# dalcinl/PetIGA

Hardware: NVIDIA B200
Metric: assembled_Mnnz_per_s (higher is better)
Workload: dtype f64

## Files before the change

### petiga_b200/csrc/pc_api.cu

```cuda
#include <dlfcn.h>

#include <sched.h>

#include <algorithm>
#include <cctype>
#include <cstdio>
#include <cstdio>
#include <cstring>
#include <string>
#include <vector>

#include "pc_plan.h"

namespace pc {

namespace {
typedef int (*nvtx_push_t)(const char*);
typedef int (*nvtx_pop_t)(void);
nvtx_push_t g_nvtx_push = nullptr;
nvtx_pop_t g_nvtx_pop = nullptr;
int g_nvtx_state = 0;
const char* const kSlotNames[PETIGA_NSLOTS] = {"IGAComputeVector", "IGAComputeMatrix", "IGAComputeSystem", "IGAComputeFunction", "IGAComputeJacobian",
                                               "IGAComputeIFunction", "IGAComputeIJacobian", "IGAComputeIEFunction", "IGAComputeIEJacobian",
                                               "IGAComputeRHSFunction", "IGAComputeRHSJacobian", "IGAComputeI2Function", "IGAComputeI2Jacobian"};
// ... 169 lines not shown
    part[2 * blockIdx.x] = x; part[2 * blockIdx.x + 1] = y;
  }
}

__global__ void __launch_bounds__(256) dfma_peak_kernel(double* out, int iters, double a, double b) {
  double x0 = threadIdx.x, x1 = x0 + 1, x2 = x0 + 2, x3 = x0 + 3, x4 = x0 + 4, x5 = x0 + 5, x6 = x0 + 6, x7 = x0 + 7;
  for (int i = 0; i < iters; i++) {
#pragma unroll
    for (int k = 0; k < 8; k++) {
      x0 = fma(x0, a, b); x1 = fma(x1, a, b); x2 = fma(x2, a, b); x3 = fma(x3, a, b);
      x4 = fma(x4, a, b); x5 = fma(x5, a, b); x6 = fma(x6, a, b); x7 = fma(x7, a, b);
    }
  }
  const double s = ((x0 + x1) + (x2 + x3)) + ((x4 + x5) + (x6 + x7));
  if (s == 12345.678) out[0] = s;
}

}

using namespace pc;

extern "C" {

int petiga_cuda_version(void) { return PETIGA_CUDA_VERSION; }

const char* petiga_cuda_strerror(int code) {
  switch (code) {
    case PETIGA_CUDA_OK: return "success";
    case PETIGA_CUDA_ERR_ARG: return "invalid argument";
    case PETIGA_CUDA_ERR_ORDER: return "operation called out of order";
    case PETIGA_CUDA_ERR_SUP: return "configuration not supported by the device path";
    case PETIGA_CUDA_ERR_MEM: return "out of memory";
    case PETIGA_CUDA_ERR_CUDA: return "CUDA runtime error";
    case PETIGA_CUDA_ERR_NODEVICE: return "no CUDA device (libpetiga_cuda has no CPU fallback)";
    case PETIGA_CUDA_ERR_NCCL: return "NCCL error";
  }
  return "unknown error";
}

const char* petiga_cuda_last_error(void) { return g_last_error.c_str(); }

int petiga_cuda_device_count(int* count) {
  int n = 0;
  cudaError_t e = cudaGetDeviceCount(&n);
  if (count) *count = (e == cudaSuccess) ? n : 0;
  if (e != cudaSuccess) return cuda_fail(e, "cudaGetDeviceCount");
  return n > 0 ? 0 : PETIGA_CUDA_ERR_NODEVICE;
}

int petiga_cuda_plan_create(petiga_cuda_plan** plan, const petiga_cuda_space* sp, int rank, int nranks, void* nccl_comm,
                            void* stream, int device) {
  if (!plan || !sp) return PETIGA_CUDA_ERR_ARG;
  *plan = nullptr;
  int ndev = 0;
  int rc = petiga_cuda_device_count(&ndev);
  if (rc) { if (g_last_error.empty()) set_error("no CUDA device; libpetiga_cuda has no CPU fallback"); return rc; }
  if (device < 0 || device >= ndev) { set_error("bad device ordinal"); return PETIGA_CUDA_ERR_ARG; }
  petiga_cuda_plan* P = new (std::nothrow) petiga_cuda_plan();
  if (!P) return PETIGA_CUDA_ERR_MEM;
  memset(&P->bc, 0, sizeof(P->bc));
  rc = build_layout(*sp, rank, nranks, P->L);
  if (rc) { set_error(P->L.error); delete P; return rc; }
  if (sp->order < 1 || sp->order > 4) { set_error("order must be in [1,4]"); delete P; return PETIGA_CUDA_ERR_ARG; }
  P->order = sp->order;
  P->device = device;
  P->nccl = nccl_comm;
  auto bail = [&](int code) { petiga_cuda_plan_destroy(P); return code; };
  if (cudaSetDevice(device) != cudaSuccess) return bail(cuda_fail(cudaGetLastError(), "cudaSetDevice"));
  if (stream) P->stream = (cudaStream_t)stream;
  else {
    cudaError_t e = cudaStreamCreateWithFlags(&P->stream, cudaStreamNonBlocking);
    if (e != cudaSuccess) return bail(cuda_fail(e, "cudaStreamCreate"));
    P->own_stream = true;
  }
  cudaDeviceGetAttribute(&P->num_sms, cudaDevAttrMultiProcessorCount, device);
  cudaEventCreate(&P->ev0);
  cudaEventCreate(&P->ev1);
  const Layout& L = P->L;
  for (int d = 0; d < 3; d++) {
    const AxisLayout& a = L.ax[d];
    DevAxis& da = P->dax[d];
    const size_t nq = (size_t)a.nel * a.nqp;
    if (!sp->value[d] || !sp->weight[d] || !sp->point[d] || !sp->detJac[d]) { set_error("missing basis tables"); return bail(PETIGA_CUDA_ERR_ARG); }
    double *v, *w, *pt, *dj; int *off, *W, *lo, *simp; uint32_t* seg;
    if ((rc = upload(P, sp->value[d], nq * (a.p + 1) * 5, &v))) return bail(rc);
    if ((rc = upload(P, sp->weight[d], nq, &w))) return bail(rc);
    if ((rc = upload(P, sp->point[d], nq, &pt))) return bail(rc);
    if ((rc = upload(P, sp->detJac[d], (size_t)a.nel, &dj))) return bail(rc);
    if ((rc = upload(P, sp->offset[d], (size_t)a.nel, &off))) return bail(rc);
    if ((rc = upload(P, a.W.data(), a.W.size(), &W))) return bail(rc);
    if ((rc = upload(P, a.lo.data(), a.lo.size(), &lo))) return bail(rc);
    if ((rc = upload(P, a.seg.data(), a.seg.size(), &seg))) return bail(rc);
    if ((rc = upload(P, a.simple.data(), a.simple.size(), &simp))) return bail(rc);
    da.value = v; da.weight = w; da.point = pt; da.detJac = dj; da.offset = off; da.W = W; da.lo = lo; da.seg = seg; da.simple = simp;
    da.nel = a.nel; da.nqp = a.nqp; da.nen = a.p + 1; da.p = a.p; da.gs = a.gs; da.gw = a.gw; da.es = a.es; da.ew = a.ew;
    da.periodic = a.periodic; da.nnp = a.nnp;
    P->detJac_h[d].assign(sp->detJac[d], sp->detJac[d] + a.nel);
    if ((rc = upload(P, L.rowG[d].data(), L.rowG[d].size(), &P->d_rowG[d]))) return bail(rc);
    if ((rc = upload(P, a.first.data(), a.first.size(), &P->d_first[d]))) return bail(rc);
    if ((rc = upload(P, a.own.data(), a.own.size(), &P->d_own[d]))) return bail(rc);
    if ((rc = upload(P, a.box_ls.data(), a.box_ls.size(), &P->d_box_ls[d]))) return bail(rc);
    if ((rc = upload(P, a.box_lw.data(), a.box_lw.size(), &P->d_box_lw[d]))) return bail(rc);
  }
  if ((rc = upload(P, L.localrow.data(), L.localrow.size(), &P->d_localrow))) return bail(rc);
  if ((rc = upload(P, L.rowbase.data(), L.rowbase.size(), &P->d_rowbase))) return bail(rc);
  if ((rc = upload(P, L.rank_start.data(), L.rank_start.size(), &P->d_rank_start))) return bail(rc);
  if (L.nranks > 1) {
    const size_t nl = (size_t)L.nloc * L.dof;
    if ((rc = upload<double>(P, nullptr, nl, &P->d_rhs_loc))) return bail(rc);
    if ((rc = upload<double>(P, nullptr, nl, &P->d_U_loc))) return bail(rc);
    if ((rc = upload<double>(P, nullptr, nl, &P->d_V_loc))) return bail(rc);
    if ((rc = upload<double>(P, nullptr, nl, &P->d_W_loc))) return bail(rc);
    std::vector<int> rows;
    std::vector<int64_t> offs;
    P->recv_row_off.clear();
    for (auto& r : L.recv) {
      P->recv_row_off.push_back(rows.size());
      rows.insert(rows.end(), r.rows.begin(), r.rows.end());
      int64_t o = 0;
      for (int row : r.rows) { offs.push_back(o); o += L.rowbase[row + 1] - L.rowbase[row]; }
    }
    P->recv_row_off.push_back(rows.size());
    if ((rc = upload(P, rows.data(), rows.size(), &P->d_recv_rows))) return bail(rc);
    if ((rc = upload(P, offs.data(), offs.size(), &P->d_recv_off))) return bail(rc);
  }
  cudaError_t e = cudaStreamSynchronize(P->stream);
  if (e != cudaSuccess) return bail(cuda_fail(e, "plan upload"));
  *plan = P;
  return 0;
}

int petiga_cuda_plan_destroy(petiga_cuda_plan* P) {
  if (!P) return 0;
  cudaSetDevice(P->device);
  if (P->stream) cudaStreamSynchronize(P->stream);
  for (void* d : P->allocs) cudaFree(d);
  for (int b = 0; b < 2; b++) { cudaFree(P->d_rowptr[b]); cudaFree(P->d_colidx[b]); }
  cudaFree(P->d_X); cudaFree(P->d_W); cudaFree(P->d_fixtable); cudaFree(P->d_ghost_values); cudaFree(P->d_recv);
  cudaFree(P->d_scalar); cudaFree(P->d_sf3_dprime); cudaFree(P->d_solve_work); cudaFree(P->d_solve_xfull); cudaFree(P->d_values_own); cudaFree(P->d_rhs_own); cudaFree(P->d_U_own); cudaFree(P->d_V_own);
  if (P->h_pinned) cudaFreeHost(P->h_pinned);
  if (P->ev0) cudaEventDestroy(P->ev0);
  if (P->ev1) cudaEventDestroy(P->ev1);
  if (P->own_stream && P->stream) cudaStreamDestroy(P->stream);
  delete P;
  return 0;
}

int petiga_cuda_set_option(petiga_cuda_plan* P, const char* name, double value) {
  if (!P || !name) return PETIGA_CUDA_ERR_ARG;
  if (!strcmp(name, "path")) { int v = (int)value; if (v < 0 || v > 2) return PETIGA_CUDA_ERR_ARG; P->path = v; return 0; }
  if (!strcmp(name, "scatter")) { P->scatter = (int)value; return 0; }
  if (!strcmp(name, "quad_impl")) { int v = (int)value; if (v < -1 || v > 3) return PETIGA_CUDA_ERR_ARG; P->quad_impl = v; return 0; }
  if (!strcmp(name, "kron_minb_rows")) { P->kron_minb_rows = (int)value; P->config_version++; return 0; }
  if (!strcmp(name, "kron_bulk")) { P->kron_bulk = value != 0; P->config_version++; return 0; }
  if (!strcmp(name, "sf3_static")) { P->sf3_static = value != 0; return 0; }
  if (!strcmp(name, "sf3_variant")) { int v = (int)value; if (v < 0 || v > 1) return PETIGA_CUDA_ERR_ARG; P->sf3_variant = v; return 0; }
  set_error(std::string("unknown option ") + name);
  return PETIGA_CUDA_ERR_ARG;
}

int petiga_cuda_get_stat(petiga_cuda_plan* P, const char* name, double* value) {
  if (!P || !name || !value) return PETIGA_CUDA_ERR_ARG;
  if (!strcmp(name, "launches")) { *value = (double)P->launches; return 0; }
  if (!strcmp(name, "last_path")) { *value = (double)P->last_path; return 0; }
  if (!strcmp(name, "last_impl")) { *value = (double)P->last_impl; return 0; }
  if (!strcmp(name, "last_sf3_static")) { *value = (double)P->last_sf3_static; return 0; }
  if (!strcmp(name, "last_sf3_variant")) { *value = (double)P->last_sf3_variant; return 0; }
  if (!strcmp(name, "last_kernel_ms")) { *value = P->last_kernel_ms; return 0; }
  if (!strcmp(name, "last_flops")) { *value = P->last_flops; return 0; }
  if (!strcmp(name, "num_sms")) { *value = P->num_sms; return 0; }
  if (!strcmp(name, "nghostrows")) { *value = P->L.nghostrows; return 0; }
  if (!strcmp(name, "nnz_loc")) { *value = (double)P->L.nnz_loc; return 0; }
  return PETIGA_CUDA_ERR_ARG;
}

int petiga_cuda_set_geometry(petiga_cuda_plan* P, int nsd, const double* X, const double* W) {
  if (!P) return PETIGA_CUDA_ERR_ARG;
  PC_CUDA(cudaSetDevice(P->device));
  PC_CUDA(cudaStreamSynchronize(P->stream));
  cudaFree(P->d_X); cudaFree(P->d_W);
  P->d_X = P->d_W = nullptr;
  P->config_version++;
  if (!X) return 0;
  if (nsd != P->L.dim) { set_error("geometry: nsd must equal dim on the device path (manifolds unsupported)"); return PETIGA_CUDA_ERR_SUP; }
  const size_t ng = P->L.localrow.size();
  PC_CUDA(cudaMalloc(&P->d_X, ng * nsd * sizeof(double)));
  PC_CUDA(cudaMemcpy(P->d_X, X, ng * nsd * sizeof(double), cudaMemcpyHostToDevice));
  if (W) {
    PC_CUDA(cudaMalloc(&P->d_W, ng * sizeof(double)));
    PC_CUDA(cudaMemcpy(P->d_W, W, ng * sizeof(double), cudaMemcpyHostToDevice));
  }
  return 0;
}

int petiga_cuda_set_bc(petiga_cuda_plan* P, const petiga_cuda_bc* bc) {
  if (!P) return PETIGA_CUDA_ERR_ARG;
  PC_CUDA(cudaSetDevice(P->device));
  PC_CUDA(cudaStreamSynchronize(P->stream));
  cudaFree(P->d_fixtable);
  P->d_fixtable = nullptr;
  P->has_bc = false;
  P->config_version++;
  memset(&P->bc, 0, sizeof(P->bc));
  if (!bc) return 0;
  for (int d = 0; d < 3; d++)
    for (int s = 0; s < 2; s++) {
      if (bc->vcount[d][s] < 0 || bc->vcount[d][s] > 64 || bc->lcount[d][s] < 0 || bc->lcount[d][s] > 64) return PETIGA_CUDA_ERR_ARG;
      if (d < P->L.dim && (bc->vcount[d][s] || bc->lcount[d][s])) P->has_bc = true;
    }
  for (int d = 0; d < 3; d++)
    for (int s = 0; s < 2; s++) {
      for (int k = 0; k < bc->vcount[d][s]; k++) {
        const int f = bc->vfield[d][s][k];
        if (f < 0) { memset(&P->bc, 0, sizeof(P->bc)); P->has_bc = false; set_error("set_bc: negative field index"); return PETIGA_CUDA_ERR_ARG; }
        int pos = -1;
        for (int j = 0; j < P->bc.vcount[d][s]; j++) if (P->bc.vfield[d][s][j] == f) pos = j;
        if (pos < 0) pos = P->bc.vcount[d][s]++;
        P->bc.vfield[d][s][pos] = f; P->bc.vvalue[d][s][pos] = bc->vvalue[d][s][k];
      }
      for (int k = 0; k < bc->lcount[d][s]; k++) {
        const int f = bc->lfield[d][s][k];
        if (f < 0) { memset(&P->bc, 0, sizeof(P->bc)); P->has_bc = false; set_error("set_bc: negative field index"); return PETIGA_CUDA_ERR_ARG; }
        int pos = -1;
        for (int j = 0; j < P->bc.lcount[d][s]; j++) if (P->bc.lfield[d][s][j] == f) pos = j;
        if (pos < 0) pos = P->bc.lcount[d][s]++;
        P->bc.lfield[d][s][pos] = f; P->bc.lvalue[d][s][pos] = bc->lvalue[d][s][k];
      }
    }
  P->bc.fixtableU = nullptr;
  if (bc->fixtableU) {
    const size_t n = P->L.localrow.size() * P->L.dof;
    PC_CUDA(cudaMalloc(&P->d_fixtable, n * sizeof(double)));
    PC_CUDA(cudaMemcpy(P->d_fixtable, bc->fixtableU, n * sizeof(double), cudaMemcpyHostToDevice));
  }
  return 0;
}

int petiga_cuda_set_fixtable_device(petiga_cuda_plan* P, const double* table_own) {
  if (!P) return PETIGA_CUDA_ERR_ARG;
  PC_CUDA(cudaSetDevice(P->device));
  PC_CUDA(cudaStreamSynchronize(P->stream));
  cudaFree(P->d_fixtable);
  P->d_fixtable = nullptr;
  P->config_version++;
  if (!table_own) return 0;
  const Layout& L = P->L;
  const size_t ng = L.localrow.size();
  PC_CUDA(cudaMalloc(&P->d_fixtable, ng * L.dof * sizeof(double)));
  const double* loc = table_own;
  double* tmp = nullptr;
  if (L.nranks > 1) {
    PC_CUDA(cudaMalloc(&tmp, (size_t)L.nloc * L.dof * sizeof(double)));
    int rc = halo_state(P, table_own, tmp);
    if (rc) { cudaFree(tmp); return rc; }
    loc = tmp;
  }
  const int blocks = (int)std::min<size_t>((ng * L.dof + 255) / 256, (size_t)P->num_sms * 8);
  fixtable_scatter_kernel<<<std::max(blocks, 1), 256, 0, P->stream>>>(P->d_localrow, loc, P->d_fixtable, ng, L.dof);
  PC_CUDA(cudaGetLastError());
  P->launches++;
  PC_CUDA(cudaStreamSynchronize(P->stream));
  cudaFree(tmp);
  return 0;
}

int petiga_cuda_form_select(petiga_cuda_plan* P, int slot, int form_id, const double* params, int nparams) {
  if (P && slot >= 0 && slot < PETIGA_NSLOTS && form_id == -1) {
    P->slots[slot].form = -1;
    P->config_version++;
    return 0;
  }
  if (!P || slot < 0 || slot >= PETIGA_NSLOTS || form_id < 0 || form_id >= PETIGA_NFORMS || nparams < 0 || nparams > kMaxPrm) {
    set_error("form_select: bad slot / form / nparams");
    return PETIGA_CUDA_ERR_ARG;
  }
  FormInfo fi = form_info(form_id, slot, P->L.dim, P->L.dof);
  if (!fi.valid) { set_error("form_select: this built-in form does not provide that slot for this dim/dof (PETSC_ERR_SUP)"); return PETIGA_CUDA_ERR_SUP; }
  P->slots[slot].form = form_id;
  P->config_version++;
  memset(P->slots[slot].prm, 0, sizeof(P->slots[slot].prm));
  for (int k = 0; k < nparams; k++) P->slots[slot].prm[k] = params[k];
  return 0;
}

int petiga_cuda_plan_sizes(petiga_cuda_plan* P, int* nown, int* nghost, int64_t* nnzb) {
  if (!P) return PETIGA_CUDA_ERR_ARG;
  if (nown) *nown = P->L.nown;
  if (nghost) *nghost = (int)P->L.localrow.size();
  if (nnzb) *nnzb = P->L.nnz_own;
  return 0;
}

int petiga_cuda_plan_lgmap_host(petiga_cuda_plan* P, int* lgmap) {
  if (!P || !lgmap) return PETIGA_CUDA_ERR_ARG;
  memcpy(lgmap, P->L.lgmap.data(), P->L.lgmap.size() * sizeof(int));
  return 0;
}

int petiga_cuda_plan_pattern(petiga_cuda_plan* P, int block, int* nrows, int64_t* nnz, const int** d_rowptr, const int** d_colidx) {
  if (!P || (block != 0 && block != 1)) return PETIGA_CUDA_ERR_ARG;
  const Layout& L = P->L;
  const int bs = block ? 1 : L.dof;
  const int64_t n = L.nnz_own * bs * bs;
  if (n > INT32_MAX) { set_error("pattern: more than 2^31-1 nonzeros on one rank; use the block (BAIJ) layout or more ranks"); return PETIGA_CUDA_ERR_SUP; }
  PC_CUDA(cudaSetDevice(P->device));
  if (!P->d_rowptr[block]) {
    std::vector<int> rp((size_t)L.nown * bs + 1);
// ... 378 lines not shown
```

### petiga_b200/csrc/pc_kron.cu

```cuda
#include <algorithm>
#include <cstdlib>
#include <cstring>

#include "pc_plan.h"

namespace pc {

namespace {

constexpr int kMaxTerms = 40;
constexpr int kKronP = 4;
constexpr int kMaxWW = (2 * kKronP + 1) * (2 * kKronP + 1);
constexpr int kStageCap = 32 * 16 + 192;

struct KronTerm { unsigned char ij, rs0, rs1, rs2; double c; };
struct KronVTerm { unsigned char i, r0, r1, r2; double c; };

struct KronParams {
  const double* M[3];
  const double* mv[3];
  const int* nsup[3];
  const double* lsum[3];
  const double* rsum[3];
  const int* first[3];
  const int* Wg[3];
  const int* lo[3];
  const uint32_t* seg[3];
  const int* simp[3];
  int ls[3], lw[3], gs[3], nnp[3], periodic[3];
  const int64_t* rowbase;
  const int* localrow;
  const double* fixtable;
  int gw[3];
  int dim, dof, block, slot, simple, wfull0;
  int nterms, nvterms, rsmask0;
  int fast_lo, fast_hi;
  int rsmask_ij[9];
  int ncombo;
  unsigned char combo_rs0[36], combo_ij[36], combo_first[37];
  signed char slotA[9], slotB[9];
  int two_slot;
  int minb_rows;
  int bulk;
  KronTerm terms[kMaxTerms];
  KronVTerm vterms[8];
  FixSide bc[3][2];
  int any_bc;
  double* values;
  double* rhs;
};

__device__ __forceinline__ int wrapi(int i, int n) { return i < 0 ? n + i : (i >= n ? i % n : i); }

__global__ void kron_1d_kernel(DevAxis ax, const int* __restrict__ first, double* __restrict__ M, double* __restrict__ mv,
                               int* __restrict__ nsup, double* __restrict__ lsum) {
  const int nnp = ax.nnp, nen = ax.nen, nq = ax.nqp;
  const int t = blockIdx.x * blockDim.x + threadIdx.x;
  const int total = nnp * kMaxW * 4;
  if (t < total) {
    const int rs = t / (nnp * kMaxW), rem = t - rs * nnp * kMaxW, i = rem / kMaxW, c = rem - i * kMaxW;
    const int r = rs >> 1, s = rs & 1;
    const int col = wrapi(first[i] + c, nnp);
    double acc = 0.0;
    const bool exists = c <= 2 * ax.p && (ax.periodic || first[i] + c < nnp);
    for (int e = 0; e < (exists ? ax.nel : 0); e++) {
      int a = -1, b = -1;
      for (int l = 0; l < nen; l++) {
        int node = wrapi(ax.offset[e] + l, nnp);
        if (node == i) a = l;
        if (node == col) b = l;
      }
      if (a < 0 || b < 0) continue;
      const double J = ax.detJac[e];
      double se = 0.0;
      for (int q = 0; q < nq; q++) {
        const double* va = ax.value + ((size_t)(e * nq + q) * nen + a) * 5;
        const double* vb = ax.value + ((size_t)(e * nq + q) * nen + b) * 5;
        se += (ax.weight[e * nq + q] * J) * va[r] * vb[s];
      }
      acc += se;
    }
    M[t] = acc;
  }
  if (t < nnp * 2) {
    const int r = t / nnp, i = t - r * nnp;
    double acc = 0.0, ls = 0.0;
    int cnt = 0;
    for (int e = 0; e < ax.nel; e++) {
      int a = -1;
      for (int l = 0; l < nen; l++) if (wrapi(ax.offset[e] + l, nnp) == i) a = l;
      if (a < 0) continue;
      const double J = ax.detJac[e];
      double se = 0.0;
      for (int q = 0; q < nq; q++) se += (ax.weight[e * nq + q] * J) * ax.value[((size_t)(e * nq + q) * nen + a) * 5 + r];
      acc += se;
      cnt++;
      ls += J / (double)nen;
    }
    mv[t] = acc;
    if (r == 0) { nsup[i] = cnt; lsum[i] = ls; }
  }
}

__global__ void kron_rowsum_kernel(const double* __restrict__ M, double* __restrict__ rsum, int nnp) {
  const int t = blockIdx.x * blockDim.x + threadIdx.x;
  if (t >= 4 * nnp) return;
  double acc = 0.0;
  for (int c = 0; c < kMaxW; c++) acc += M[(size_t)t * kMaxW + c];
  rsum[t] = acc;
}

template <int DOF>
__device__ __forceinline__ void node_fix(const KronParams& kp, int c0, int c1, int c2, bool fixed[DOF], double val[DOF]) {
#pragma unroll
  for (int c = 0; c < DOF; c++) { fixed[c] = false; val[c] = 0.0; }
  const int code[3] = {c0, c1, c2};
#pragma unroll
  for (int d = 0; d < 3; d++) {
    if (d >= kp.dim || !code[d]) continue;
    const FixSide& fs = kp.bc[d][code[d] - 1];
    for (int k = 0; k < fs.vcount; k++)
#pragma unroll
      for (int c = 0; c < DOF; c++)
        if (fs.vfield[k] == c) { fixed[c] = true; val[c] = fs.vvalue[k]; }
  }
}

__device__ __forceinline__ int bcode(int col, int nnp, int periodic) { return periodic ? 0 : ((col == 0) ? 1 : ((col == nnp - 1) ? 2 : 0)); }

template <int DOF, int PF, int MINB>
__global__ void __launch_bounds__(256, MINB) kron_rows_kernel(const __grid_constant__ KronParams kp) {
  extern __shared__ __align__(16) double dynstage[];
  __shared__ double G[4][DOF * DOF][kMaxWW];
  __shared__ int jkinfo[kMaxWW];
  __shared__ int jkp1[kMaxWW];
  __shared__ double jkval[kMaxWW];
  __shared__ double Gm[2][kMaxWW];
  __shared__ double Hs[2];
  __shared__ int fast_ctr;
  const int pencil = (int)blockIdx.x;
  const int Aj = kp.ls[1] + pencil % kp.lw[1], Ak = kp.ls[2] + pencil / kp.lw[1];
  const int gj = Aj - kp.gs[1], gk = Ak - kp.gs[2];
  const int Wj = kp.Wg[1][gj], Wk = kp.Wg[2][gk], Wjk = Wj * Wk;
  const int fj = kp.first[1][Aj], fk = kp.first[2][Ak];
  const bool fixing = kp.any_bc && kp.slot == PETIGA_SLOT_SYSTEM;
  __shared__ double sM[2][4][kMaxW];
  __shared__ uint32_t sSeg[2][kMaxW];
  for (int t = threadIdx.x; t < 2 * 4 * kMaxW; t += blockDim.x) {
    const int d = t / (4 * kMaxW), rs = (t / kMaxW) & 3, cc = t % kMaxW;
    (&sM[0][0][0])[t] = kp.M[1 + d][((size_t)rs * kp.nnp[1 + d] + (d ? Ak : Aj)) * kMaxW + cc];
  }
  if (threadIdx.x < 2 * kMaxW) {
    const int d = threadIdx.x / kMaxW, cc = threadIdx.x % kMaxW;
    sSeg[d][cc] = kp.seg[1 + d][(d ? gk : gj) * kMaxW + cc];
  }
  for (int t = threadIdx.x; t < 4 * DOF * DOF * kMaxWW; t += blockDim.x) (&G[0][0][0])[t] = 0.0;
  if (threadIdx.x == 0) fast_ctr = 0;
  __syncthreads();
  for (int w = threadIdx.x; w < kp.ncombo * Wjk; w += blockDim.x) {
    const int k = w / Wjk, t = w - k * Wjk, cj = t % Wj, ck = t / Wj;
    double acc = 0.0;
    for (int n = kp.combo_first[k]; n < kp.combo_first[k + 1]; n++) {
      const KronTerm tm = kp.terms[n];
      acc += tm.c * sM[0][tm.rs1][cj] * sM[1][tm.rs2][ck];
    }
    G[kp.combo_rs0[k]][kp.combo_ij[k]][t] = acc;
  }
  bool jk_boundary = false;
  for (int t = threadIdx.x; t < Wjk; t += blockDim.x) {
    const int cj = t % Wj, ck = t / Wj;
    int info = bcode(fj + cj, kp.nnp[1], kp.periodic[1]) | (bcode(fk + ck, kp.nnp[2], kp.periodic[2]) << 2);
    if (cj == Aj - fj && ck == Ak - fk) info |= 16;
    int p1 = 0;
    {
      const uint32_t s1 = sSeg[0][cj], s2 = sSeg[1][ck];
      const int Bj = s1 & 255, Sj = (s1 >> 8) & 255, Lj = (s1 >> 16) & 255;
      const int Bk = s2 & 255, Sk = (s2 >> 8) & 255, Lk = (s2 >> 16) & 255;
      p1 = Bk * Wj + Sk * Bj;
      info |= (Sk * Sj) << 8;
      info |= (Lk * Sj + Lj) << 16;
    }
    if (DOF == 1 && fixing && (info & 15)) {
      bool f[1]; double fv[1];
      node_fix<1>(kp, 0, info & 3, (info >> 2) & 3, f, fv);
      if (f[0]) { info |= 32; jkval[t] = fv[0]; }
    }
    jkinfo[t] = info;
    jkp1[t] = p1;
  }
  jk_boundary = fixing && ((!kp.periodic[1] && ((fj == 0 && kp.bc[1][0].vcount) || (fj + Wj == kp.nnp[1] && kp.bc[1][1].vcount))) ||
                           (!kp.periodic[2] && ((fk == 0 && kp.bc[2][0].vcount) || (fk + Wk == kp.nnp[2] && kp.bc[2][1].vcount))));
  __syncthreads();
  const int lane = threadIdx.x & 31, warp = threadIdx.x >> 5, nwarps = blockDim.x >> 5;
  const bool want_mat = kp.values != nullptr, want_vec = kp.rhs != nullptr;
  const int rcj = bcode(Aj, kp.nnp[1], kp.periodic[1]), rck = bcode(Ak, kp.nnp[2], kp.periodic[2]);
  const int lw0 = kp.lw[0], ls0 = kp.ls[0], gs0 = kp.gs[0], nnp0 = kp.nnp[0], per0 = kp.periodic[0];
// ... 299 lines not shown
          if (DOF == 1) kp.values[(size_t)(base + pos)] = v[0];
          else {
#pragma unroll
            for (int i = 0; i < DOF; i++)
#pragma unroll
              for (int j = 0; j < DOF; j++) {
                size_t off;
                if (kp.block) off = (size_t)(base + pos) * DOF * DOF + j * DOF + i;
                else off = (size_t)base * DOF * DOF + (size_t)i * W * DOF + (size_t)pos * DOF + j;
                kp.values[off] = v[i * DOF + j];
              }
          }
        }
        }
        if (staged) {
          const int e0 = cjk0 * Wi, ne = min(ngrp * Wi, W - e0);
          if (act) {
#pragma unroll
            for (int i = 0; i < DOF; i++)
#pragma unroll
              for (int j = 0; j < DOF; j++) stg[lane * DOF * DOF + j * DOF + i] = v[i * DOF + j];
          }
          __syncwarp();
          double* dst = kp.values + (size_t)(base + e0) * DOF * DOF;
          for (int t = lane; t < ne * DOF * DOF; t += 32) dst[t] = stg[t];
          __syncwarp();
        }
      }
    }
    if (want_vec) {
      if (col_boundary) {
#pragma unroll
        for (int c = 0; c < DOF; c++) {
          double r = racc[c];
#pragma unroll
          for (int o = 16; o > 0; o >>= 1) r += __shfl_xor_sync(0xffffffffu, r, o);
          racc[c] = r;
        }
      }
      if (lane == 0) {
#pragma unroll
        for (int c = 0; c < DOF; c++) {
          double F = 0.0;
          for (int n = 0; n < kp.nvterms; n++) {
            const KronVTerm vt = kp.vterms[n];
            if (vt.i != c) continue;
            F += vt.c * kp.mv[0][vt.r0 * kp.nnp[0] + Ai] * kp.mv[1][vt.r1 * kp.nnp[1] + Aj] * kp.mv[2][vt.r2 * kp.nnp[2] + Ak];
          }
          if (row_boundary) {
            const int rcode[3] = {rci, rcj, rck};
            for (int d = 0; d < kp.dim; d++) {
              if (!rcode[d]) continue;
              const FixSide& fs = kp.bc[d][rcode[d] - 1];
              if (!fs.lcount) continue;
              double A = 1.0;
              if (kp.dim > 1) {
                const int An[3] = {Ai, Aj, Ak};
                for (int e2 = 0; e2 < kp.dim; e2++) if (e2 != d) A *= kp.lsum[e2][An[e2]];
                A *= (kp.dim == 2) ? 2 : 4;
              }
              for (int k = 0; k < fs.lcount; k++) if (fs.lfield[k] == c) F += fs.lvalue[k] * A;
            }
          }
          F += racc[c];
          if (rfix[c]) F = nelem * rval[c];
          kp.rhs[(size_t)lr * DOF + c] = F;
        }
      }
    }
  }
  if constexpr (DOF > 1 && PF > 0) {
    if (blk_fast) {
      constexpr int NSPLIT = 2;
      constexpr int WIC = 2 * PF + 1, WJKC = WIC * WIC, KT = (WIC * WJKC * DD + 31) / 32, KH = (KT + NSPLIT - 1) / NSPLIT;
      constexpr int NACV = (WIC * DD * 2 + 31) / 32;
      const int WR = WIC * Wjk, NV = WR * DD;
      const int h = warp % NSPLIT, pairi = warp / NSPLIT, npair = nwarps / NSPLIT;
      double gA[KH], gB[KH];
      int aoff[KH];
#pragma unroll
      for (int k = 0; k < KH; k++) {
        const int t = 32 * (h * KH + k) + lane;
        gA[k] = gB[k] = 0.0; aoff[k] = 0;
        if (t < NV) {
          int blk, i, j;
          if (kp.block) { blk = t / DD; const int e = t - blk * DD; j = e / DOF; i = e - j * DOF; }
          else { i = t / (WR * DOF); const int r2 = t - i * (WR * DOF); blk = r2 / DOF; j = r2 - blk * DOF; }
          const int ij = i * DOF + j, cjk = blk / WIC, ci = blk - cjk * WIC;
          if (kp.slotA[ij] >= 0) gA[k] = G[kp.slotA[ij]][ij][cjk];
          if (kp.slotB[ij] >= 0) gB[k] = G[kp.slotB[ij]][ij][cjk];
          aoff[k] = (ci * DD + (kp.block ? j * DOF + i : ij)) * 2;
        }
      }
      int acg[NACV];
#pragma unroll
      for (int k = 0; k < NACV; k++) {
        acg[k] = -1;
        const int t = lane + 32 * k;
        if (t < WIC * DD * 2) {
          const int ci = t / (DD * 2), r2 = t - ci * (DD * 2), q = r2 >> 1;
          const int ij = kp.block ? (q % DOF) * DOF + q / DOF : q;
          const int rs = (r2 & 1) ? kp.slotB[ij] : kp.slotA[ij];
          if (rs >= 0) acg[k] = rs * nnp0 * kMaxW + ci;
        }
      }
      double* acs = dynstage + warp * kStageCap + 32 * DD;
      double acv[NACV];
      int il = fast_lo + pairi;
#pragma unroll
      for (int k = 0; k < NACV; k++) acv[k] = (il < kp.fast_hi && acg[k] >= 0) ? __ldg(M0 + acg[k] + (size_t)(ls0 + il) * kMaxW) : 0.0;
      int64_t base_n = il < kp.fast_hi ? __ldg(rowbase + lr0 + il) : 0;
      for (; il < kp.fast_hi; il += npair) {
        const int Ai = ls0 + il, lr = il + lr0;
        const int64_t base = base_n;
        if (il + npair < kp.fast_hi) base_n = __ldg(rowbase + lr + npair);
#pragma unroll
        for (int k = 0; k < NACV; k++) { const int t = lane + 32 * k; if (t < WIC * DD * 2) acs[t] = acv[k]; }
        const int iln = il + npair;
#pragma unroll
        for (int k = 0; k < NACV; k++) acv[k] = (iln < kp.fast_hi && acg[k] >= 0) ? __ldg(M0 + acg[k] + (size_t)(ls0 + iln) * kMaxW) : 0.0;
        __syncwarp();
        double* __restrict__ dst = values + (size_t)base * DD + 32 * (h * KH) + lane;
        constexpr int KB = (KH + 2) / 3;
#pragma unroll
        for (int b3 = 0; b3 < 3; b3++) {
          double2 a2[KB];
#pragma unroll
          for (int kk = 0; kk < KB; kk++) { const int k = b3 * KB + kk; if (k < KH) a2[kk] = *reinterpret_cast<const double2*>(acs + aoff[k]); }
#pragma unroll
          for (int kk = 0; kk < KB; kk++) {
            const int k = b3 * KB + kk;
            if (k < KH && 32 * (h * KH + k) + lane < NV) dst[32 * k] = fma(a2[kk].y, gB[k], a2[kk].x * gA[k]);
          }
        }
        __syncwarp();
        if (want_vec && h == 0 && lane == 0) {
#pragma unroll
          for (int cc = 0; cc < DOF; cc++) {
            double F = 0.0;
            for (int n = 0; n < kp.nvterms; n++) {
              const KronVTerm vt = kp.vterms[n];
              if (vt.i != cc) continue;
              F += vt.c * kp.mv[0][vt.r0 * nnp0 + Ai] * kp.mv[1][vt.r1 * kp.nnp[1] + Aj] * kp.mv[2][vt.r2 * kp.nnp[2] + Ak];
            }
            rhs[(size_t)lr * DOF + cc] = F;
          }
        }
      }
    }
  }
  if (PF > 0 && pencil_fast) {
    constexpr int WIC = 2 * PF + 1, WJKC = WIC * WIC, NGRP = 32 / WIC, NITER = (WJKC + NGRP - 1) / NGRP, OSTEP = NGRP * WIC, RW = WIC * WJKC, R = 4;
    const int64_t base_lo = __ldg(rowbase + lr0 + fast_lo);
    const double* __restrict__ g0 = jk_boundary ? &Gm[0][grpF] : &G[0][0][grpF];
    const double* __restrict__ g3 = jk_boundary ? &Gm[1][grpF] : &G[3][0][grpF];
    const double H0 = jk_boundary ? Hs[0] : 0.0, H3 = jk_boundary ? Hs[1] : 0.0;
    for (;;) {
      int grab = 0;
      if (lane == 0) grab = atomicAdd(&fast_ctr, 1);
      grab = __shfl_sync(0xffffffffu, grab, 0);
      const int il = fast_lo + grab * R;
      if (il >= kp.fast_hi) break;
      if (kp.bulk) {
        double* sb = dynstage + warp * (R * RW + 4);
        const int64_t gstart = base_lo + (int64_t)(il - fast_lo) * RW;
        const int par = (int)(gstart & 1);
        asm volatile("cp.async.bulk.wait_group.read 0;" ::: "memory");
        __syncwarp();
        if (grpF < NGRP) {
          double a0[R], a3[R];
#pragma unroll
          for (int r = 0; r < R; r++) {
            a0[r] = __ldg(M0 + (size_t)(ls0 + il + r) * kMaxW + ciF);
            a3[r] = __ldg(M0 + ((size_t)3 * nnp0 + ls0 + il + r) * kMaxW + ciF);
          }
          double* __restrict__ rowp = sb + par + offF;
#pragma unroll
          for (int k = 0; k < NITER; k++)
            if ((k + 1) * NGRP <= WJKC || grpF + k * NGRP < WJKC) {
              const double x0 = g0[k * NGRP], x3 = g3[k * NGRP];
#pragma unroll
              for (int r = 0; r < R; r++) rowp[r * RW + k * OSTEP] = fma(a3[r], x3, a0[r] * x0);
            }
        }
        asm volatile("fence.proxy.async.shared::cta;" ::: "memory");
        __syncwarp();
        if (lane == 0) {
          const uint32_t nbytes = (uint32_t)(R * RW - 2 * par) * 8u;
          asm volatile("cp.async.bulk.global.shared::cta.bulk_group [%0], [%1], %2;"
                       ::"l"(__cvta_generic_to_global(values + gstart + par)), "r"((uint32_t)__cvta_generic_to_shared(sb + 2 * par)), "r"(nbytes) : "memory");
          asm volatile("cp.async.bulk.commit_group;" ::: "memory");
          if (par) { values[gstart] = sb[1]; values[gstart + R * RW - 1] = sb[R * RW]; }
        }
      } else
      if (grpF < NGRP) {
        double a0[R], a3[R];
#pragma unroll
        for (int r = 0; r < R; r++) {
          a0[r] = __ldg(M0 + (size_t)(ls0 + il + r) * kMaxW + ciF);
          a3[r] = __ldg(M0 + ((size_t)3 * nnp0 + ls0 + il + r) * kMaxW + ciF);
        }
        double* __restrict__ rowp = values + base_lo + (int64_t)(il - fast_lo) * RW + offF;
#pragma unroll
        for (int k = 0; k < NITER; k++)
          if ((k + 1) * NGRP <= WJKC || grpF + k * NGRP < WJKC) {
            const double x0 = g0[k * NGRP], x3 = g3[k * NGRP];
#pragma unroll
            for (int r = 0; r < R; r++) rowp[r * RW + k * OSTEP] = fma(a3[r], x3, a0[r] * x0);
          }
      }
      if (want_vec && lane < R) {
        const int Ai = ls0 + il + lane;
        double F;
        if (vsimple) F = vjk * __ldg(mv0 + Ai);
        else {
          F = 0.0;
          for (int n = 0; n < kp.nvterms; n++) {
            const KronVTerm vt = kp.vterms[n];
            F += vt.c * kp.mv[0][vt.r0 * nnp0 + Ai] * kp.mv[1][vt.r1 * kp.nnp[1] + Aj] * kp.mv[2][vt.r2 * kp.nnp[2] + Ak];
          }
        }
        if (jk_boundary) F -= __ldg(kp.rsum[0] + Ai) * H0 + __ldg(kp.rsum[0] + (size_t)3 * nnp0 + Ai) * H3;
        rhs[lr0 + il + lane] = F;
      }
    }
    if (kp.bulk) asm volatile("cp.async.bulk.wait_group 0;" ::: "memory");
  }
}

template <int DIM, int DOF>
void host_terms(int form, int slot, const double* prm, const FormInfo& fi, KronParams& kp) {
  const int NA = fi.mc1 - fi.mc0, NV = fi.vc1 - fi.vc0;
  std::vector<double> C((size_t)DOF * DOF * std::max(NA, 1) * std::max(NA, 1), 0.0), fv((size_t)DOF * std::max(NV, 1), 0.0);
  QPoint q;
  memset(&q, 0, sizeof(q));
  form_coefficients<DIM, DOF>(form, slot, prm, 0.0, 0.0, q, NA, NV, NA ? C.data() : nullptr, (NV && fi.constant_f) ? fv.data() : nullptr);
  kp.nterms = kp.nvterms = kp.rsmask0 = 0;
  for (int k = 0; k < 9; k++) kp.rsmask_ij[k] = 0;
  for (int i = 0; i < DOF; i++)
    for (int j = 0; j < DOF; j++)
      for (int al = 0; al < NA; al++)
        for (int be = 0; be < NA; be++) {
          double c = C[(((size_t)i * DOF + j) * NA + al) * NA + be];
          if (c == 0.0) continue;
          KronTerm t;
          const int ca = al + fi.mc0, cb = be + fi.mc0;
          unsigned char rs[3];
          for (int d = 0; d < 3; d++) rs[d] = (unsigned char)(((ca == 1 + d) ? 2 : 0) + ((cb == 1 + d) ? 1 : 0));
          t.ij = (unsigned char)(i * DOF + j); t.rs0 = rs[0]; t.rs1 = rs[1]; t.rs2 = rs[2]; t.c = c;
          if (kp.nterms < kMaxTerms) kp.terms[kp.nterms] = t;
          kp.nterms++;
          kp.rsmask0 |= 1 << rs[0];
          kp.rsmask_ij[i * DOF + j] |= 1 << rs[0];
        }
  for (int i = 0; i < DOF; i++)
    for (int al = 0; al < NV; al++) {
      double c = fv[(size_t)i * NV + al];
      if (c == 0.0) continue;
      const int ca = al + fi.vc0;
      KronVTerm t;
      t.i = (unsigned char)i; t.r0 = (ca == 1); t.r1 = (ca == 2); t.r2 = (ca == 3); t.c = c;
      if (kp.nvterms < 8) kp.vterms[kp.nvterms] = t;
      kp.nvterms++;
    }
}

}

static int launch_kron_kernel(petiga_cuda_plan* P, const KronParams& kp) {
  const Layout& L = P->L;
  const int blocks = L.ax[1].lw * L.ax[2].lw;
  int threads = std::min(256, std::max(32, ((L.ax[0].lw + 0) * 32)));
  if (const char* e = getenv("PETIGA_KRON_THREADS")) threads = std::max(32, std::min(256, atoi(e) / 32 * 32));
  int pf = L.ax[0].p;
  for (int d = 1; d < L.dim; d++) if (L.ax[d].p != pf) pf = 0;
  if (L.dim < 3 || (L.dof != 1 && pf > 2)) pf = 0;
  size_t dyn = L.dof > 1 ? (size_t)(threads / 32) * kStageCap * sizeof(double) : 0;
  if (L.dof == 1 && kp.bulk && pf > 0) dyn = (size_t)(threads / 32) * (4 * (2 * pf + 1) * (2 * pf + 1) * (2 * pf + 1) + 4) * sizeof(double);
  const int minb = L.dof > 1 ? 2 : (L.ax[0].lw >= kp.minb_rows ? 3 : 4);
#define KL(DOF_, PF_, MB_) if (L.dof == DOF_ && pf == PF_ && minb == MB_) { \
    if (dyn) PC_CUDA(cudaFuncSetAttribute(kron_rows_kernel<DOF_, PF_, MB_>, cudaFuncAttributeMaxDynamicSharedMemorySize, (int)dyn)); \
    kron_rows_kernel<DOF_, PF_, MB_><<<blocks, threads, dyn, P->stream>>>(kp); }
  KL(1, 0, 3) KL(1, 1, 3) KL(1, 2, 3) KL(1, 3, 3) KL(1, 4, 3) KL(1, 0, 4) KL(1, 1, 4) KL(1, 2, 4) KL(1, 3, 4) KL(1, 4, 4)
  KL(2, 0, 2) KL(3, 0, 2) KL(2, 1, 2) KL(2, 2, 2) KL(3, 1, 2) KL(3, 2, 2)
#undef KL
  PC_CUDA(cudaGetLastError());
  P->launches++;
  return 0;
}

bool kron_applicable(const petiga_cuda_plan* P, int slot, int form) {
  const Layout& L = P->L;
  if (slot != PETIGA_SLOT_VECTOR && slot != PETIGA_SLOT_MATRIX && slot != PETIGA_SLOT_SYSTEM) return false;
  if (P->d_X) return false;
  FormInfo fi = form_info(form, slot, L.dim, L.dof);
  if (!fi.valid || !fi.mat_const) return false;
  if (!fi.constant_f) {
    if (slot == PETIGA_SLOT_VECTOR) return false;
    if (slot == PETIGA_SLOT_SYSTEM && P->has_bc) return false;
  }
  if (L.dof > 3) return false;
  for (int d = 0; d < L.dim; d++) if (L.ax[d].p > kKronP) return false;
  if (P->d_fixtable && L.nranks > 1) return false;
  for (int d = 0; d < L.dim; d++)
    if (L.ax[d].periodic && L.ax[d].nnp < 2 * L.ax[d].p + 1) return false;
  return true;
}

int launch_kronecker(petiga_cuda_plan* P, int slot, int block, double* values, double* rhs) {
  const Layout& L = P->L;
  const int form = P->slots[slot].form;
  FormInfo fi = form_info(form, slot, L.dim, L.dof);
  if (!P->d_kronrow[0]) {
    for (int d = 0; d < 3; d++) {
      const int nnp = L.ax[d].nnp;
      void* buf = nullptr;
      const size_t nM = (size_t)4 * nnp * kMaxW, nmv = (size_t)2 * nnp;
      PC_CUDA(cudaMalloc(&buf, (nM + nmv + nnp + (size_t)4 * nnp) * sizeof(double) + (size_t)nnp * sizeof(int)));
      P->allocs.push_back(buf);
      P->d_kronrow[d] = (double*)buf;
      double* M = (double*)buf; double* mv = M + nM; double* lsum = mv + nmv; double* rsum = lsum + nnp; int* nsup = (int*)(rsum + (size_t)4 * nnp);
      const int total = (int)nM;
      kron_1d_kernel<<<(total + 127) / 128, 128, 0, P->stream>>>(P->dax[d], P->d_first[d], M, mv, nsup, lsum);
      PC_CUDA(cudaGetLastError());
      kron_rowsum_kernel<<<(4 * nnp + 127) / 128, 128, 0, P->stream>>>(M, rsum, nnp);
      PC_CUDA(cudaGetLastError());
      P->launches += 2;
    }
  }
  if (P->kron_cache.size() == sizeof(KronParams) && P->kron_cache_slot == slot && P->kron_cache_block == block &&
      P->kron_cache_version == P->config_version) {
    KronParams kc;
    memcpy(&kc, P->kron_cache.data(), sizeof(kc));
    kc.values = values; kc.rhs = rhs;
    return launch_kron_kernel(P, kc);
  }
  KronParams kp;
  memset(&kp, 0, sizeof(kp));
  bool simple = (L.nranks == 1);
  for (int d = 0; d < 3; d++) {
    const int nnp = L.ax[d].nnp;
    const size_t nM = (size_t)4 * nnp * kMaxW, nmv = (size_t)2 * nnp;
    kp.M[d] = P->d_kronrow[d]; kp.mv[d] = kp.M[d] + nM; kp.lsum[d] = kp.mv[d] + nmv; kp.rsum[d] = kp.lsum[d] + nnp; kp.nsup[d] = (const int*)(kp.rsum[d] + (size_t)4 * nnp);
    kp.first[d] = P->d_first[d]; kp.Wg[d] = P->dax[d].W; kp.lo[d] = P->dax[d].lo; kp.seg[d] = P->dax[d].seg; kp.simp[d] = P->dax[d].simple;
    kp.ls[d] = L.ax[d].ls; kp.lw[d] = L.ax[d].lw; kp.gs[d] = L.ax[d].gs; kp.gw[d] = L.ax[d].gw; kp.nnp[d] = nnp; kp.periodic[d] = L.ax[d].periodic;
    if (L.ax[d].periodic) simple = false;
  }
  kp.rowbase = P->d_rowbase; kp.localrow = P->d_localrow; kp.fixtable = P->d_fixtable;
  kp.dim = L.dim; kp.dof = L.dof; kp.block = block; kp.slot = slot; kp.simple = simple; kp.wfull0 = 2 * L.ax[0].p + 1;
  kp.bulk = P->kron_bulk;
  kp.minb_rows = P->kron_minb_rows;
  kp.values = values; kp.rhs = rhs;
  const double* prm = P->slots[slot].prm;
#define HT(DIM_, DOF_) if (L.dim == DIM_ && L.dof == DOF_) host_terms<DIM_, DOF_>(form, slot, prm, fi, kp);
  HT(1, 1) HT(1, 2) HT(1, 3) HT(2, 1) HT(2, 2) HT(2, 3) HT(3, 1) HT(3, 2) HT(3, 3)
#undef HT
  if (kp.nterms > kMaxTerms || kp.nvterms > 8) { set_error("separable path: too many coefficient terms"); return PETIGA_CUDA_ERR_SUP; }
  {
    std::stable_sort(kp.terms, kp.terms + kp.nterms, [](const KronTerm& a, const KronTerm& b) { return a.rs0 * 16 + a.ij < b.rs0 * 16 + b.ij; });
    kp.ncombo = 0;
    for (int n = 0; n < kp.nterms; n++) {
      if (n == 0 || kp.terms[n].rs0 != kp.terms[n - 1].rs0 || kp.terms[n].ij != kp.terms[n - 1].ij) {
        kp.combo_rs0[kp.ncombo] = kp.terms[n].rs0; kp.combo_ij[kp.ncombo] = kp.terms[n].ij; kp.combo_first[kp.ncombo] = (unsigned char)n;
        kp.ncombo++;
      }
    }
    kp.combo_first[kp.ncombo] = (unsigned char)kp.nterms;
  }
  kp.two_slot = 1;
  for (int ij = 0; ij < 9; ij++) {
    kp.slotA[ij] = kp.slotB[ij] = -1;
    int n = 0;
    for (int rs = 0; rs < 4; rs++)
      if ((kp.rsmask_ij[ij] >> rs) & 1) { if (n == 0) kp.slotA[ij] = (signed char)rs; else if (n == 1) kp.slotB[ij] = (signed char)rs; n++; }
    if (n > 2) kp.two_slot = 0;
  }
  if (slot == PETIGA_SLOT_SYSTEM && P->has_bc)
    for (int d = 0; d < L.dim; d++)
      for (int s = 0; s < 2; s++) {
        FixSide& fs = kp.bc[d][s];
        for (int k = 0; k < P->bc.vcount[d][s]; k++) {
          int c = P->bc.vfield[d][s][k];
          if (c >= L.dof || fs.vcount >= kMaxDof) continue;
          fs.vfield[fs.vcount] = c; fs.vvalue[fs.vcount] = P->bc.vvalue[d][s][k]; fs.vcount++;
        }
        for (int k = 0; k < P->bc.lcount[d][s]; k++) {
          int c = P->bc.lfield[d][s][k];
          if (c >= L.dof || fs.lcount >= kMaxDof) continue;
          fs.lfield[fs.lcount] = c; fs.lvalue[fs.lcount] = P->bc.lvalue[d][s][k]; fs.lcount++;
        }
        if (!L.ax[d].periodic && (fs.vcount || fs.lcount)) kp.any_bc = 1;
      }
  {
    const AxisLayout& a0 = L.ax[0];
    const bool fixing0 = kp.any_bc && slot == PETIGA_SLOT_SYSTEM && !a0.periodic;
    int best_lo = 0, best_hi = 0, run_lo = -1;
    for (int il = 0; il <= a0.lw; il++) {
      bool ok = false;
      if (il < a0.lw) {
        const int Ai = a0.ls + il, gi = Ai - a0.gs, Wi = a0.W[gi], fi = a0.first[Ai];
        ok = (Wi == 2 * a0.p + 1) && a0.simple[gi];
        if (ok && fixing0 && (Ai == 0 || Ai == a0.nnp - 1 || fi == 0 || fi + Wi == a0.nnp)) ok = false;
      }
      if (ok) { if (run_lo < 0) run_lo = il; }
      else if (run_lo >= 0) { if (il - run_lo > best_hi - best_lo) { best_lo = run_lo; best_hi = il; } run_lo = -1; }
    }
    kp.fast_lo = best_lo;
    kp.fast_hi = best_lo + (best_hi - best_lo) / 4 * 4;
  }
  P->kron_cache.resize(sizeof(KronParams));
  memcpy(P->kron_cache.data(), &kp, sizeof(kp));
  P->kron_cache_slot = slot; P->kron_cache_block = block; P->kron_cache_version = P->config_version;
  return launch_kron_kernel(P, kp);
}

}
```

### petiga_b200/csrc/pc_plan.h

```cpp
#pragma once
#include <cuda_runtime.h>

#include <string>
#include <vector>

#include "pc_device.h"

struct petiga_cuda_plan {
  pc::Layout L;
  int device = 0;
  cudaStream_t stream = nullptr;
  bool own_stream = false;
  void* nccl = nullptr;
  int order = 1;

  std::vector<double> detJac_h[3];
  std::vector<int> first_h[3];

  pc::DevAxis dax[3];
  std::vector<void*> allocs;
  int* d_localrow = nullptr;
  int64_t* d_rowbase = nullptr;
  int* d_rowG[3] = {nullptr, nullptr, nullptr};
  int* d_first[3] = {nullptr, nullptr, nullptr};
  int* d_own[3] = {nullptr, nullptr, nullptr};
  int* d_box_ls[3] = {nullptr, nullptr, nullptr};
  int* d_box_lw[3] = {nullptr, nullptr, nullptr};
  int* d_rank_start = nullptr;
  double* d_kron1d[3] = {nullptr, nullptr, nullptr};
  double* d_kronrow[3] = {nullptr, nullptr, nullptr};
  double* d_sfpp[3] = {nullptr, nullptr, nullptr};
  double* d_sf3pp[3] = {nullptr, nullptr, nullptr};
  double* d_solve_work = nullptr; size_t solve_work_cap = 0;
  double* d_solve_xfull = nullptr; size_t solve_xfull_cap = 0;
  double* d_sf3_dprime = nullptr; size_t sf3_dprime_cap = 0;

  int* d_rowptr[2] = {nullptr, nullptr};
  int* d_colidx[2] = {nullptr, nullptr};

  double* d_X = nullptr;
  double* d_W = nullptr;
  double* d_fixtable = nullptr;
  double* d_bnd_value[3][2] = {{nullptr, nullptr}, {nullptr, nullptr}, {nullptr, nullptr}};
  double bnd_point[3][2] = {{0, 0}, {0, 0}, {0, 0}};
  int visit[3][2] = {{0, 0}, {0, 0}, {0, 0}};
  double* d_face_dS[3][2] = {{nullptr, nullptr}, {nullptr, nullptr}, {nullptr, nullptr}};
  long face_version[3][2] = {{-1, -1}, {-1, -1}, {-1, -1}};
  petiga_cuda_bc bc;
  bool has_bc = false;
  double* d_ghost_values = nullptr; size_t ghost_values_cap = 0;
  double* d_rhs_loc = nullptr;
  double* d_U_loc = nullptr;
  double* d_V_loc = nullptr;
  double* d_W_loc = nullptr;
  double* d_recv = nullptr; size_t recv_cap = 0;
  int* d_recv_rows = nullptr;
  int64_t* d_recv_off = nullptr;
  std::vector<size_t> recv_row_off;
  double* h_pinned = nullptr; size_t h_pinned_cap = 0;
  double* d_values_own = nullptr; size_t values_own_cap = 0;
  double* d_rhs_own = nullptr;
  double* d_U_own = nullptr;
  double* d_V_own = nullptr;
  double* d_scalar = nullptr; size_t scalar_cap = 0;

  struct Slot { int form = -1; double prm[pc::kMaxPrm] = {0}; } slots[PETIGA_NSLOTS];
  int path = PETIGA_PATH_AUTO;
  int scatter = 0;
  std::vector<unsigned char> kron_cache;
  int kron_cache_slot = -1, kron_cache_block = -1;
  long kron_cache_version = -1, config_version = 0;
  int kron_minb_rows = 100;
  int kron_bulk = 0;
  int sf3_variant = 0;
  int last_sf3_variant = 0;
  int sf3_static = 1, last_sf3_static = 0;
  int quad_impl = -1;
  long launches = 0;
  int last_path = 0;
  int last_impl = 0;
  double last_kernel_ms = 0;
  double last_flops = 0;
  cudaEvent_t ev0 = nullptr, ev1 = nullptr;
  int num_sms = 148;
};

namespace pc {
void set_error(const std::string& msg);
void nvtx_push(int slot);
void nvtx_pop();
int cuda_fail(cudaError_t e, const char* what);
#define PC_CUDA(call)                                              \
  do {                                                             \
    cudaError_t _e = (call);                                       \
    if (_e != cudaSuccess) return pc::cuda_fail(_e, #call);        \
  } while (0)

int launch_quadrature(petiga_cuda_plan* P, const KParams& base);
int launch_quadrature_sf(petiga_cuda_plan* P, const KParams& base);
int launch_quadrature_vec3(petiga_cuda_plan* P, const KParams& base);
int launch_quadrature_sf3(petiga_cuda_plan* P, const KParams& base);
int launch_quadrature_gen(petiga_cuda_plan* P, const KParams& base);
bool kron_applicable(const petiga_cuda_plan* P, int slot, int form);
int launch_kronecker(petiga_cuda_plan* P, int slot, int block, double* values, double* rhs);
int exchange_ghost_rows(petiga_cuda_plan* P, int block, double* values, double* rhs, bool mat, bool vec);
int halo_state(petiga_cuda_plan* P, const double* U_own, double* U_loc);
int nccl_load();
int allgather_owned(petiga_cuda_plan* P, const double* owned, double* full);
int allreduce_sum(petiga_cuda_plan* P, double* d_buf, int n);
void nvtx_push(const char* name);
int launch_boundary_pass(petiga_cuda_plan* P, int slot, int form, const double* prm, double* rhs, bool apply_fix);
}
```

Before: 750,800.

## Replace bulk-copy staging with sector-aligned direct stores in PF=3 Kronecker fast path

Removes the optional cp.async.bulk shared-memory staging path and its option. For the p=3 scalar pencil fast path, lanes now write directly to global values in 28-element pieces aligned to 32-byte sectors, using an alignment offset phi. Lanes that cross a row boundary pull coefficients from the next row, and the first and last partial pieces are handled specially. The goal is fully coalesced, sector-aligned stores without staging, at the cost of more complex index arithmetic and extra loads for the look-ahead row.

Measured after the change: 804,100 (median of 6 runs). +7.1%, better.

```diff
diff --git a/petiga_b200/csrc/pc_api.cu b/petiga_b200/csrc/pc_api.cu
--- a/petiga_b200/csrc/pc_api.cu
+++ b/petiga_b200/csrc/pc_api.cu
@@ -345,7 +345,6 @@
   if (!strcmp(name, "scatter")) { P->scatter = (int)value; return 0; }
   if (!strcmp(name, "quad_impl")) { int v = (int)value; if (v < -1 || v > 3) return PETIGA_CUDA_ERR_ARG; P->quad_impl = v; return 0; }
   if (!strcmp(name, "kron_minb_rows")) { P->kron_minb_rows = (int)value; P->config_version++; return 0; }
-  if (!strcmp(name, "kron_bulk")) { P->kron_bulk = value != 0; P->config_version++; return 0; }
   if (!strcmp(name, "sf3_static")) { P->sf3_static = value != 0; return 0; }
   if (!strcmp(name, "sf3_variant")) { int v = (int)value; if (v < 0 || v > 1) return PETIGA_CUDA_ERR_ARG; P->sf3_variant = v; return 0; }
   set_error(std::string("unknown option ") + name);
diff --git a/petiga_b200/csrc/pc_kron.cu b/petiga_b200/csrc/pc_kron.cu
--- a/petiga_b200/csrc/pc_kron.cu
+++ b/petiga_b200/csrc/pc_kron.cu
@@ -41,7 +41,6 @@
   signed char slotA[9], slotB[9];
   int two_slot;
   int minb_rows;
-  int bulk;
   KronTerm terms[kMaxTerms];
   KronVTerm vterms[8];
   FixSide bc[3][2];
@@ -647,48 +646,45 @@
   if (PF > 0 && pencil_fast) {
     constexpr int WIC = 2 * PF + 1, WJKC = WIC * WIC, NGRP = 32 / WIC, NITER = (WJKC + NGRP - 1) / NGRP, OSTEP = NGRP * WIC, RW = WIC * WJKC, R = 4;
     const int64_t base_lo = __ldg(rowbase + lr0 + fast_lo);
-    const double* __restrict__ g0 = jk_boundary ? &Gm[0][grpF] : &G[0][0][grpF];
-    const double* __restrict__ g3 = jk_boundary ? &Gm[1][grpF] : &G[3][0][grpF];
+    const double* __restrict__ g0 = jk_boundary ? Gm[0] : G[0][0];
+    const double* __restrict__ g3 = jk_boundary ? Gm[1] : G[3][0];
     const double H0 = jk_boundary ? Hs[0] : 0.0, H3 = jk_boundary ? Hs[1] : 0.0;
+    constexpr int NG = 4, PIECE = NG * WIC, NPC = R * WJKC / NG;
+    static_assert(PF != 3 || (PIECE % 4 == 0 && PIECE <= 32 && (R * WJKC) % NG == 0), "aligned pieces need whole sectors and whole runs");
+    const int phi = (int)((0 - (reinterpret_cast<uintptr_t>(values + base_lo) >> 3)) & 3);
+    const int q = phi + lane, s0 = q / WIC, ciA = q - s0 * WIC;
     for (;;) {
       int grab = 0;
       if (lane == 0) grab = atomicAdd(&fast_ctr, 1);
       grab = __shfl_sync(0xffffffffu, grab, 0);
       const int il = fast_lo + grab * R;
       if (il >= kp.fast_hi) break;
-      if (kp.bulk) {
-        double* sb = dynstage + warp * (R * RW + 4);
-        const int64_t gstart = base_lo + (int64_t)(il - fast_lo) * RW;
-        const int par = (int)(gstart & 1);
-        asm volatile("cp.async.bulk.wait_group.read 0;" ::: "memory");
-        __syncwarp();
-        if (grpF < NGRP) {
-          double a0[R], a3[R];
+      if constexpr (PF == 3) {
+        if (lane < PIECE) {
+          const bool more = il + R < kp.fast_hi;
+          double a0[R + 1], a3[R + 1];
 #pragma unroll
           for (int r = 0; r < R; r++) {
-            a0[r] = __ldg(M0 + (size_t)(ls0 + il + r) * kMaxW + ciF);
-            a3[r] = __ldg(M0 + ((size_t)3 * nnp0 + ls0 + il + r) * kMaxW + ciF);
-          }
-          double* __restrict__ rowp = sb + par + offF;
-#pragma unroll
-          for (int k = 0; k < NITER; k++)
-            if ((k + 1) * NGRP <= WJKC || grpF + k * NGRP < WJKC) {
-              const double x0 = g0[k * NGRP], x3 = g3[k * NGRP];
-#pragma unroll
-              for (int r = 0; r < R; r++) rowp[r * RW + k * OSTEP] = fma(a3[r], x3, a0[r] * x0);
-            }
-        }
-        asm volatile("fence.proxy.async.shared::cta;" ::: "memory");
-        __syncwarp();
-        if (lane == 0) {
-          const uint32_t nbytes = (uint32_t)(R * RW - 2 * par) * 8u;
-          asm volatile("cp.async.bulk.global.shared::cta.bulk_group [%0], [%1], %2;"
-                       ::"l"(__cvta_generic_to_global(values + gstart + par)), "r"((uint32_t)__cvta_generic_to_shared(sb + 2 * par)), "r"(nbytes) : "memory");
-          asm volatile("cp.async.bulk.commit_group;" ::: "memory");
-          if (par) { values[gstart] = sb[1]; values[gstart + R * RW - 1] = sb[R * RW]; }
-        }
-      } else
-      if (grpF < NGRP) {
+            a0[r] = __ldg(M0 + (size_t)(ls0 + il + r) * kMaxW + ciA);
+            a3[r] = __ldg(M0 + ((size_t)3 * nnp0 + ls0 + il + r) * kMaxW + ciA);
+          }
+          a0[R] = a3[R] = 0.0;
+          if (more && s0 == NG) {
+            a0[R] = __ldg(M0 + (size_t)(ls0 + il + R) * kMaxW + ciA);
+            a3[R] = __ldg(M0 + ((size_t)3 * nnp0 + ls0 + il + R) * kMaxW + ciA);
+          }
+          double* __restrict__ dst = values + base_lo + (int64_t)(il - fast_lo) * RW + q;
+          if (grab == 0 && s0 == NG) dst[-PIECE] = fma(a3[0], g3[0], a0[0] * g0[0]);
+#pragma unroll
+          for (int n = 0; n < NPC; n++) {
+            const int rb = NG * n / WJKC;
+            const bool up = NG * n + NG >= (rb + 1) * WJKC && NG * n + s0 >= (rb + 1) * WJKC;
+            const int cjk = s0 + NG * n - WJKC * rb - (up ? WJKC : 0);
+            const double x0 = up ? a0[rb + 1] : a0[rb], x3 = up ? a3[rb + 1] : a3[rb];
+            if (n < NPC - 1 || !up || more) dst[n * PIECE] = fma(x3, g3[cjk], x0 * g0[cjk]);
+          }
+        }
+      } else if (grpF < NGRP) {
         double a0[R], a3[R];
 #pragma unroll
         for (int r = 0; r < R; r++) {
@@ -699,7 +695,7 @@
 #pragma unroll
         for (int k = 0; k < NITER; k++)
           if ((k + 1) * NGRP <= WJKC || grpF + k * NGRP < WJKC) {
-            const double x0 = g0[k * NGRP], x3 = g3[k * NGRP];
+            const double x0 = g0[grpF + k * NGRP], x3 = g3[grpF + k * NGRP];
 #pragma unroll
             for (int r = 0; r < R; r++) rowp[r * RW + k * OSTEP] = fma(a3[r], x3, a0[r] * x0);
           }
@@ -719,7 +715,6 @@
         rhs[lr0 + il + lane] = F;
       }
     }
-    if (kp.bulk) asm volatile("cp.async.bulk.wait_group 0;" ::: "memory");
   }
 }
 
@@ -771,7 +766,6 @@
   for (int d = 1; d < L.dim; d++) if (L.ax[d].p != pf) pf = 0;
   if (L.dim < 3 || (L.dof != 1 && pf > 2)) pf = 0;
   size_t dyn = L.dof > 1 ? (size_t)(threads / 32) * kStageCap * sizeof(double) : 0;
-  if (L.dof == 1 && kp.bulk && pf > 0) dyn = (size_t)(threads / 32) * (4 * (2 * pf + 1) * (2 * pf + 1) * (2 * pf + 1) + 4) * sizeof(double);
   const int minb = L.dof > 1 ? 2 : (L.ax[0].lw >= kp.minb_rows ? 3 : 4);
 #define KL(DOF_, PF_, MB_) if (L.dof == DOF_ && pf == PF_ && minb == MB_) { \
     if (dyn) PC_CUDA(cudaFuncSetAttribute(kron_rows_kernel<DOF_, PF_, MB_>, cudaFuncAttributeMaxDynamicSharedMemorySize, (int)dyn)); \
@@ -843,7 +837,6 @@
   }
   kp.rowbase = P->d_rowbase; kp.localrow = P->d_localrow; kp.fixtable = P->d_fixtable;
   kp.dim = L.dim; kp.dof = L.dof; kp.block = block; kp.slot = slot; kp.simple = simple; kp.wfull0 = 2 * L.ax[0].p + 1;
-  kp.bulk = P->kron_bulk;
   kp.minb_rows = P->kron_minb_rows;
   kp.values = values; kp.rhs = rhs;
   const double* prm = P->slots[slot].prm;
diff --git a/petiga_b200/csrc/pc_plan.h b/petiga_b200/csrc/pc_plan.h
--- a/petiga_b200/csrc/pc_plan.h
+++ b/petiga_b200/csrc/pc_plan.h
@@ -71,7 +71,6 @@
   int kron_cache_slot = -1, kron_cache_block = -1;
   long kron_cache_version = -1, config_version = 0;
   int kron_minb_rows = 100;
-  int kron_bulk = 0;
   int sf3_variant = 0;
   int last_sf3_variant = 0;
   int sf3_static = 1, last_sf3_static = 0;
```
